# Kkuntal990/video-to-video-diffusion

Hardware: AMD Instinct MI355X
Metric: ddim_steps_per_sec (higher is better)
Workload: dtype bf16; 1 GPU; DDIM-50 step (U-Net eval + update) on latent [1, 8, 48, 128, 128] = 8->48 slices @512x512, effective 264.66M U-Net (128x(1,2,4,4), latent 8), one volume per GPU, hipGraph-captured step; volumes_per_gpu=1, parallelism=dp1, full=False, finite_outputs=True

## Files before the change

video-to-video-diffusion_amd/csrc/conv_mfma.hip:

```cpp
#include <type_traits>
#include "conv3_halo_common.h"
#include "conv_plan.h"
#include <string.h>
#include <stdlib.h>
#include <math.h>


__device__ __attribute__((aligned(256))) uint32_t g_ctsi_zero_page[64];

struct ConvKParams {
    const bf16_t* x1;
    const bf16_t* x2;
    const bf16_t* w;
    const float* bias;
    void* y;
    float* colsum;
    int C1, C2, Cin;
    int Di, Hi, Wi;
    int Dr, Hr, Wr;
    int sH, sW;
    int lTH, lTW;
    int linear;
    int tilesD, tilesH, tilesW, tps, mtiles;
    int ntiles_n;
// ... 470 lines not shown
            const int co = n0 + col;
            float s1 = 0.0f, s2 = 0.0f;
#pragma unroll
            for (int i = 0; i < TM; ++i) {
#pragma unroll
                for (int r = 0; r < 16; ++r) {
                    const int row = wm * TM * 32 + i * 32 + (r & 3) + 8 * (r >> 2) + 4 * lhi;
                    float v = acc[i][j][r];
                    if (p.act == 1) v = tanhf(v);
                    const bool valid = (vbits[i] >> r) & 1u;
                    if (valid) {
                        s1 += v;
                        s2 += v * v;
                    }
                    if (p.out_mode == 0) {
                        s_tile[row * BN + col] = f32_to_bf16(v);
                    } else if (valid && co < p.Cout) {
                        reinterpret_cast<float*>(p.y)[s_rowoff[row] + (long long)co * p.osc] = v;
                    }
                }
            }
            if (want_sums) {
                s1 += __shfl_xor(s1, 32);
                s2 += __shfl_xor(s2, 32);
                if (lhi == 0) {
                    s_cs[(wm * BN + col) * 2 + 0] = s1;
                    s_cs[(wm * BN + col) * 2 + 1] = s2;
                }
            }
        }
    }
    if (p.gn_x != nullptr && tid < BN) {
        const int co = n0 + tid;
        float sc = 0.0f, sh = 0.0f;
        if (co < p.Cout) {
            const int cpg = p.Cout / p.gn_groups, g = co / cpg;
            const double* sm = p.gn_sums + ((long long)nb * p.gn_groups + g) * 2;
            const double mean = sm[0] / p.gn_count;
            double var = sm[1] / p.gn_count - mean * mean;
            if (var < 0.0) var = 0.0;
            const float rstd = (float)(1.0 / sqrt(var + (double)p.gn_eps));
            sc = p.gn_gamma[co] * rstd;
            sh = p.gn_beta[co] - (float)mean * sc;
        }
        s_cs[tid] = sc;
        s_cs[BN + tid] = sh;
    }
    __syncthreads();
    if (p.colsum != nullptr && tid < BN) {
        float t1 = 0.0f, t2 = 0.0f;
#pragma unroll
        for (int m = 0; m < WM; ++m) {
            t1 += s_cs[(m * BN + tid) * 2 + 0];
            t2 += s_cs[(m * BN + tid) * 2 + 1];
        }
        const long long tg = (long long)cls * p.mtiles + mt;
        const long long slab = (long long)p.nclass * p.mtiles * p.CoutPad;
        p.colsum[tg * p.CoutPad + n0 + tid] = t1;
        p.colsum[slab + tg * p.CoutPad + n0 + tid] = t2;
    }
    if (p.out_mode == 0) {
        constexpr int CPR = BN / 8;
        constexpr int ITER = (BM * CPR) / NTH;
        static_assert((BM * CPR) % NTH == 0, "store loop assumes whole iterations");
        bf16_t* y = reinterpret_cast<bf16_t*>(p.y);
        if (p.gn_x != nullptr) {
            uint4 hreg[ITER];
#pragma unroll
            for (int it = 0; it < ITER; ++it) {
                const int c = tid + it * NTH;
                const int row = c / CPR, cc = c - row * CPR;
                const long long off = s_rowoff[row];
                const int co = n0 + cc * 8;
                hreg[it] = (off >= 0 && co < p.Cout) ? *reinterpret_cast<const uint4*>(p.gn_x + off + co)
                                                     : make_uint4(0, 0, 0, 0);
            }
            static_assert(NTH % CPR == 0, "a thread's chunk must not depend on the iteration");
            const int cc0 = tid % CPR;
            float gsc[8], gsh[8];
            *reinterpret_cast<float4*>(gsc) = *reinterpret_cast<const float4*>(s_cs + cc0 * 8);
            *reinterpret_cast<float4*>(gsc + 4) = *reinterpret_cast<const float4*>(s_cs + cc0 * 8 + 4);
            *reinterpret_cast<float4*>(gsh) = *reinterpret_cast<const float4*>(s_cs + BN + cc0 * 8);
            *reinterpret_cast<float4*>(gsh + 4) = *reinterpret_cast<const float4*>(s_cs + BN + cc0 * 8 + 4);
            auto tail = [&](auto silu_tag) {
                constexpr bool SILU = decltype(silu_tag)::value;
#pragma unroll
                for (int it = 0; it < ITER; ++it) {
                    const int c = tid + it * NTH;
                    const int row = c / CPR, cc = c - row * CPR;
                    const long long off = s_rowoff[row];
                    const int co = n0 + cc * 8;
                    if (off >= 0 && co < p.Cout) {
                        const uint4 v = *reinterpret_cast<const uint4*>(s_tile + row * BN + cc * 8);
                        const uint4 h = hreg[it];
                        const uint32_t hw[4] = {h.x, h.y, h.z, h.w}, rw[4] = {v.x, v.y, v.z, v.w};
                        uint32_t ow[4];
#pragma unroll
                        for (int k = 0; k < 4; ++k) {
                            f32x2_t a = {__uint_as_float(hw[k] << 16), __uint_as_float(hw[k] & 0xffff0000u)};
                            a = a * f32x2_t{gsc[2 * k], gsc[2 * k + 1]} + f32x2_t{gsh[2 * k], gsh[2 * k + 1]} +
                                f32x2_t{__uint_as_float(rw[k] << 16), __uint_as_float(rw[k] & 0xffff0000u)};
                            if (SILU) a = silu2_f(a);
                            ow[k] = pack_bf16x2_v(a);
                        }
                        *reinterpret_cast<uint4*>(y + off + co) = make_uint4(ow[0], ow[1], ow[2], ow[3]);
                    }
                }
            };
            if (p.gn_silu) tail(std::true_type{});
            else tail(std::false_type{});
        } else {
            for (int c = tid; c < BM * CPR; c += NTH) {
                const int row = c / CPR, cc = c - row * CPR;
                const long long off = s_rowoff[row];
                const int co = n0 + cc * 8;
                if (off >= 0 && co < p.Cout && !(CTSI_DBG_RT(p.dbg, 1))) {
                    const uint4 v = *reinterpret_cast<const uint4*>(s_tile + row * BN + cc * 8);
                    *reinterpret_cast<uint4*>(y + off + co) = v;
                }
            }
        }
    }
#endif
}

struct PackParams {
    const float* w;
    bf16_t* out;
    int nclass, T, Cout, CoutPad, Cin, CinW, Ktot, small, kc_per_tap, lcpt;
    long long s_co, s_ci;
    int tapk[CTSI_MAX_TAPS];
};

__global__ void conv_pack_weights_kernel(const PackParams q) {
    const long long total = (long long)q.nclass * q.CoutPad * q.Ktot;
    for (long long idx = (long long)blockIdx.x * blockDim.x + threadIdx.x; idx < total;
         idx += (long long)gridDim.x * blockDim.x) {
        const int k = (int)(idx % q.Ktot);
        const long long rc = idx / q.Ktot;
        const int co = (int)(rc % q.CoutPad);
        const int cls = (int)(rc / q.CoutPad);
        int tap, ci;
        if (q.small) {
            const int g = k >> 3;
            tap = g >> q.lcpt;
            ci = ((g & ((1 << q.lcpt) - 1)) << 3) + (k & 7);
        } else {
            const int s = k >> 6;
            tap = s % q.T;
            ci = (s / q.T) * 64 + (k & 63);
        }
        float v = 0.0f;
        if (tap < q.T && ci < q.CinW && co < q.Cout)
            v = q.w[(long long)co * q.s_co + (long long)ci * q.s_ci + q.tapk[cls * q.T + tap]];
        q.out[idx] = f32_to_bf16(v);
    }
}

extern "C" int ctsi_conv_plan_pack_weights(const ctsi_conv_plan* p, const float* w, void* packed,
                                           void* stream) {
    CTSI_CHECK_ARG(p && w && packed, "ctsi_conv_plan_pack_weights: null argument");
    if (p->stem) return ctsi_conv3_stem_pack(w, packed, p->d.cout, p->CoutPad, p->CinW, stream);
    if (p->stream1) return ctsi_conv1_stream_pack(w, packed, p->d.cout, p->Cin, p->CinW, p->stream1, stream);
    const ConvFamily family = conv_family(p);
    if (family == CONV_K32)
        return ctsi_conv3_halo_k32_pack(w, packed, p->d.cout, p->CoutPad, p->Cin, p->CinW, p->BN, conv_k32_image(p),
                                        conv_k32_direct(p), stream);
    if (family == CONV_HEAD) {
        hipMemsetAsync((char*)packed + head1_bytes(p) - 1280, 0, 1280, (hipStream_t)stream);
        if (ctsi_conv3_head2_supported(p->Cin, p->d.cout)) {
            const int rc = ctsi_conv3_head2_pack(w, (char*)packed + head1_bytes(p), p->d.cout, p->Cin, p->CinW, stream);
            if (rc != CTSI_OK) return rc;
        }
        return ctsi_conv3_halo_pack(w, packed, p->d.cout, p->d.cout <= 8 ? 8 : 16, p->Cin, p->CinW, stream);
    }
    if (family == CONV_HALO32) return ctsi_conv3_halo_pack(w, packed, p->d.cout, p->CoutPad, p->Cin, p->CinW, stream);
    PackParams q;
    memset(&q, 0, sizeof(q));
    q.w = w;
    q.out = (bf16_t*)packed;
    q.nclass = p->nclass;
    q.T = p->T;
    q.Cout = p->d.cout;
    q.CoutPad = p->CoutPad;
    q.Cin = p->Cin;
    q.CinW = p->CinW;
    q.Ktot = p->Ktot;
    q.small = p->small;
    q.kc_per_tap = p->kc_per_tap;
    q.lcpt = p->lcpt;
    const long long KK = (long long)p->d.kd * p->d.kh * p->d.kw;
    if (!p->d.transposed) {
        q.s_co = (long long)p->CinW * KK;
        q.s_ci = KK;
    } else {
        q.s_ci = (long long)p->d.cout * KK;
        q.s_co = KK;
    }
    memcpy(q.tapk, p->tapk, sizeof(q.tapk));
    const long long total = (long long)q.nclass * q.CoutPad * q.Ktot;
    const int blocks = (int)((total + 255) / 256 > 4096 ? 4096 : (total + 255) / 256);
    hipLaunchKernelGGL(conv_pack_weights_kernel, dim3(blocks), dim3(256), 0, (hipStream_t)stream, q);
    CTSI_LAUNCH_CHECK();
    return CTSI_OK;
}

template <int WM, int WN, int TM, int TN>
static int launch_conv(const ConvKParams& k, int mode, int grid, hipStream_t st) {
    constexpr int BM = WM * TM * 32, BN = WN * TN * 32;
    constexpr size_t lds = 2 * (BM * 128 + BN * 128) + BM * 8 + WM * BN * 8;
    constexpr int STAGE = BM * 128 + BN * 128;
    constexpr int NSTG = STAGE <= 32768 ? 4 : (STAGE <= 49152 ? 3 : 2);
    constexpr size_t lds_ring = (size_t)NSTG * STAGE + BM * 8 + WM * BN * 8;
    static CtsiPerDeviceOnce attr_once;
    if (attr_once.first()) {
        hipFuncSetAttribute((const void*)conv_gather_mfma_kernel<WM, WN, TM, TN, 3>,
                            hipFuncAttributeMaxDynamicSharedMemorySize, (int)lds_ring);
        hipFuncSetAttribute((const void*)conv_gather_mfma_kernel<WM, WN, TM, TN, 0>,
                            hipFuncAttributeMaxDynamicSharedMemorySize, (int)lds);
        hipFuncSetAttribute((const void*)conv_gather_mfma_kernel<WM, WN, TM, TN, 1>,
                            hipFuncAttributeMaxDynamicSharedMemorySize, (int)lds);
        hipFuncSetAttribute((const void*)conv_gather_mfma_kernel<WM, WN, TM, TN, 2>,
                            hipFuncAttributeMaxDynamicSharedMemorySize, (int)lds);
    }
    const dim3 g(grid), b(WM * WN * 64);
    if (mode == 1)
        hipLaunchKernelGGL((conv_gather_mfma_kernel<WM, WN, TM, TN, 1>), g, b, lds, st, k);
    else if (mode == 3)
        hipLaunchKernelGGL((conv_gather_mfma_kernel<WM, WN, TM, TN, 3>), g, b, lds_ring, st, k);
    else if (mode == 2)
        hipLaunchKernelGGL((conv_gather_mfma_kernel<WM, WN, TM, TN, 2>), g, b, lds, st, k);
    else
        hipLaunchKernelGGL((conv_gather_mfma_kernel<WM, WN, TM, TN, 0>), g, b, lds, st, k);
    CTSI_LAUNCH_CHECK();
    return CTSI_OK;
}

extern "C" int ctsi_conv_fwd(const ctsi_conv_plan* p, const void* x1, const void* x2, const void* packed_w,
                             const float* bias, const ctsi_conv_out* o, void* stream) {
    CTSI_CHECK_ARG(p && x1 && packed_w && o && o->y, "ctsi_conv_fwd: null argument");
    CTSI_CHECK_ARG(p->d.c2 == 0 || x2 != nullptr, "ctsi_conv_fwd: plan has two sources but x2 is null");
    CTSI_CHECK_ARG(o->mode == 0 || o->mode == 1, "ctsi_conv_fwd: bad output mode %d", o->mode);
    if (o->mode == 0) {
        CTSI_CHECK_ARG(p->d.cout % 8 == 0 && o->cout_stride % 8 == 0 && o->c_off % 8 == 0 &&
                           o->cout_stride >= o->c_off + p->d.cout,
                       "ctsi_conv_fwd: bf16 output needs cout, cout_stride, c_off multiples of 8 "
                       "(cout=%d stride=%d off=%d)", p->d.cout, o->cout_stride, o->c_off);
    }
    const ConvFamily family = conv_family(p);
    CTSI_CHECK_ARG(o->act != 2 || (p->planar && o->mode == 0 && o->colsum == nullptr && o->gn_x == nullptr),
                   "ctsi_conv_fwd: the ReLU epilogue (act = 2) exists on planar (1,3,3) halo-tile plans with plain bf16 output "
                   "only (ctsi_conv_plan_form: bit 16 of out[4])");
    CTSI_CHECK_ARG(!p->planar || o->colsum == nullptr, "ctsi_conv_fwd: a planar (1,3,3) halo-tile plan writes no column sums");
    if (p->stem && o->mode == 0 && o->act == 0 && o->gn_x == nullptr) {
        StemParams q;
        memset(&q, 0, sizeof(q));
        q.x = (const bf16_t*)x1;
        q.w = (const bf16_t*)packed_w;
        q.bias = bias;
        q.y = (bf16_t*)o->y;
        q.colsum = (float*)o->colsum;
        q.cx = p->d.c1;
        q.D = p->d.di; q.H = p->d.hi; q.W = p->d.wi;
        q.Cout = p->d.cout; q.CoutPad = p->CoutPad;
        q.cout_stride = o->cout_stride; q.c_off = o->c_off;
        q.tilesD = p->tilesD; q.tilesH = p->tilesH; q.tilesW = p->tilesW; q.tps = p->tps; q.mtiles = p->mtiles;
        return ctsi_conv3_stem_launch(&q, stream);
    }
    CTSI_CHECK_ARG(!p->stem, "ctsi_conv_fwd: a one-channel stem plan writes bf16 without activation or fused tail");
    if (p->stream1) {
        CTSI_CHECK_ARG(o->mode == 0 && o->act == 0 && o->colsum == nullptr,
                       "ctsi_conv_fwd: a streaming 1x1x1 plan writes bf16 without activation or column sums");
        Conv1StreamParams q;
        memset(&q, 0, sizeof(q));
        q.x1 = (const bf16_t*)x1;
        q.x2 = (const bf16_t*)(x2 ? x2 : x1);
        q.w = (const bf16_t*)packed_w;
        q.bias = bias;
        q.h = (const bf16_t*)o->gn_x;
        q.y = (bf16_t*)o->y;
        if (o->gn_x != nullptr) {
            CTSI_CHECK_ARG(o->gn_sums && o->gn_gamma && o->gn_beta && o->gn_groups > 0 && p->d.cout % o->gn_groups == 0 &&
                               o->gn_count > 0,
                           "ctsi_conv_fwd: bad fused GroupNorm arguments (groups=%d, cout=%d)", o->gn_groups, p->d.cout);
            q.gn_sums = (const double*)o->gn_sums;
            q.gn_gamma = (const float*)o->gn_gamma;
            q.gn_beta = (const float*)o->gn_beta;
            q.gn_groups = o->gn_groups;
            q.gn_eps = o->gn_eps;
            q.gn_count = (double)o->gn_count;
            q.gn_silu = o->gn_silu;
        }
        q.C1 = p->d.c1; q.C2 = p->d.c2; q.Cout = p->d.cout;
        q.cout_stride = o->cout_stride; q.c_off = o->c_off;
        q.V = (long long)p->Do * p->Ho * p->Wo;
        return ctsi_conv1_stream_launch(&q, p->d.n, p->stream1, stream);
    }
    if (o->gn_x != nullptr) {
        CTSI_CHECK_ARG(!p->form && o->mode == 0 && o->act == 0 && o->colsum == nullptr && p->nclass == 1,
                       "ctsi_conv_fwd: the fused GroupNorm tail needs a gather-kernel plan, bf16 output, no act / colsum");
        CTSI_CHECK_ARG(o->gn_sums && o->gn_gamma && o->gn_beta && o->gn_groups > 0 && p->d.cout % o->gn_groups == 0 &&
                           o->gn_count > 0,
                       "ctsi_conv_fwd: bad fused GroupNorm arguments (groups=%d, cout=%d)", o->gn_groups, p->d.cout);
    }
    if (p->form && (family == CONV_HEAD || (o->mode == 0 && (o->act == 0 || o->act == 2)))) {
        Conv3HaloParams h;
        memset(&h, 0, sizeof(h));
        h.x1 = (const bf16_t*)x1;
        h.x2 = (const bf16_t*)(x2 ? x2 : x1);
        h.w = (const bf16_t*)packed_w;
        h.bias = bias;
        h.y = o->y;
        h.colsum = o->colsum;
        h.C1 = p->d.c1; h.C2 = p->d.c2;
        h.Di = p->d.di; h.Hi = p->d.hi; h.Wi = p->d.wi;
        h.Do = p->Do; h.Ho = p->Ho; h.Wo = p->Wo;
        h.dshift = p->dshift;
        h.tilesD = p->tilesD; h.tilesH = p->tilesH; h.tilesW = p->tilesW; h.tps = p->tps; h.mtiles = p->mtiles;
        h.ntiles_n = p->ntiles_n;
        h.nchunks = p->Cin / (family == CONV_K32 ? 16 : 32) * (p->ds ? 4 : 1);
        h.ds = p->ds;
        h.Cout = p->d.cout; h.CoutPad = p->CoutPad;
        h.cout_stride = o->cout_stride; h.c_off = o->c_off;
        {
            static const char* nts = getenv("CTSI_CONV_NT_STORE");
            const long long out_bytes = (long long)p->d.n * p->Do * p->Ho * p->Wo * o->cout_stride * 2;
            h.nt_store = nts ? atoi(nts) != 0 : out_bytes >= (128ll << 20);
        }
        {
            const char* nm = getenv("CTSI_CONV_NMAJOR");
            h.n_major = nm ? atoi(nm) : 0;
            if (p->d.transposed && !nm) h.n_major = 4;
        }
        {
            h.dbg = ctsi_debug_flags();
            h.nchunks = ctsi_debug_ksteps(h.nchunks);
        }
        {
            const char* to = getenv("CTSI_CONV_TILE_ORDER");
            h.tile_order = to ? atoi(to) : 2;
            const char* eb = getenv("CTSI_CONV_EPI_BARRIER");
            h.dbg_epi_barrier = eb ? atoi(eb) : 0;
        }
        if (family == CONV_HEAD) {
            if (p->head2 && o->colsum == nullptr)
                return ctsi_conv3_head2_launch(&h, p->d.n, (const char*)packed_w + head1_bytes(p), o->mode, o->act, o->sn, o->sc, o->sd,
                                               o->sh, o->sw, stream);
            return ctsi_conv3_head_launch(&h, p->d.cout <= 8 ? 8 : 16, o->mode, o->act, o->sn, o->sc, o->sd, o->sh, o->sw, stream);
        }
        h.tr = p->d.transposed;
        if (family == CONV_K32 && p->ksplit == 2) {
            CTSI_CHECK_ARG(o->workspace, "ctsi_conv_fwd: this plan needs ctsi_conv_out.workspace (ctsi_conv_plan_workspace_bytes)");
            const int tiles = p->mtiles * p->ntiles_n;
            h.ksplit = 2;
            h.sk_sync = (int*)o->workspace;
            h.sk_ws = (float*)((char*)o->workspace + ((size_t)tiles * 8 + 255) / 256 * 256);
        }
        if (p->planar) return ctsi_conv3_planar_k32_launch(&h, p->form->code, o->act == 2, stream);
        if (family == CONV_K32) return ctsi_conv3_halo_k32_launch(&h, p->form->code, p->BN, stream);
        return ctsi_conv3_halo_launch(&h, p->form->code, stream);
    }
    CTSI_CHECK_ARG(!p->form, "ctsi_conv_fwd: the 3x3x3 halo-tile plan supports bf16 NDHWC output without activation");
    ConvKParams k;
    memset(&k, 0, sizeof(k));
    k.x1 = (const bf16_t*)x1;
    k.x2 = (const bf16_t*)(x2 ? x2 : x1);
    k.w = (const bf16_t*)packed_w;
    k.bias = bias;
    k.y = o->y;
    k.colsum = o->colsum;
    k.C1 = p->d.c1; k.C2 = p->d.c2; k.Cin = p->Cin;
    k.Di = p->d.di; k.Hi = p->d.hi; k.Wi = p->d.wi;
    k.Dr = p->Dr; k.Hr = p->Hr; k.Wr = p->Wr;
    k.sH = p->sH; k.sW = p->sW;
    k.lTH = p->lTH; k.lTW = p->lTW;
    k.linear = p->linear;
    k.tilesD = p->tilesD; k.tilesH = p->tilesH; k.tilesW = p->tilesW; k.tps = p->tps; k.mtiles = p->mtiles;
    k.ntiles_n = p->ntiles_n;
    k.T = p->T; k.ksteps = p->ksteps; k.kc_per_tap = p->kc_per_tap; k.lcpt = p->lcpt;
    k.Cout = p->d.cout; k.CoutPad = p->CoutPad; k.Ktot = p->Ktot;
    k.Do = p->Do; k.Ho = p->Ho; k.Wo = p->Wo; k.uH = p->uH; k.uW = p->uW;
    k.nclass = p->nclass;
    k.out_mode = o->mode; k.cout_stride = o->cout_stride; k.c_off = o->c_off; k.act = o->act;
    k.osn = o->sn; k.osc = o->sc; k.osd = o->sd; k.osh = o->sh; k.osw = o->sw;
    memcpy(k.tapdelta, p->tapdelta, sizeof(k.tapdelta));
    k.NA = p->NA; k.NB = p->NB; k.NC = p->NC;
    memcpy(k.ad, p->ad, sizeof(k.ad));
    memcpy(k.bh, p->bh, sizeof(k.bh));
    memcpy(k.cw, p->cw, sizeof(k.cw));
    for (int c = 0; c < 4; ++c) { k.pH[c] = p->pH[c]; k.pW[c] = p->pW[c]; }
    int grid = p->nclass * p->mtiles * p->ntiles_n;
    if (p->gsplit >= 2 && o->workspace != nullptr && !(p->BM != 128 || p->BN != 128)) {
        const size_t tiles = (size_t)grid;
        k.ksplit = p->gsplit;
        k.sk_sync = (int*)o->workspace;
        k.sk_ws = (float*)((char*)o->workspace + (tiles * 4 + 255) / 256 * 256);
        grid *= p->gsplit;
    }
    hipStream_t st = (hipStream_t)stream;
    k.ksteps = ctsi_debug_ksteps(k.ksteps);
    k.dbg = ctsi_debug_flags();
    k.gn_x = (const bf16_t*)o->gn_x;
    k.gn_sums = o->gn_sums;
    k.gn_gamma = o->gn_gamma;
    k.gn_beta = o->gn_beta;
    k.gn_groups = o->gn_groups;
    k.gn_silu = o->gn_silu;
    k.gn_eps = o->gn_eps;
    k.gn_count = (double)o->gn_count;
    k.dshift = p->dshift;
    memcpy(k.tap_margin, p->tap_margin, sizeof(k.tap_margin));
    memcpy(k.ad_min, p->ad_min, sizeof(k.ad_min));
    int mode = p->small ? 1 : (p->fast ? 2 : 0);
    {
        const char* ring = getenv("CTSI_CONV_RING");
        const bool small_grid = grid <= 256 && !(p->BM == 256 && p->BN == 256);
        if (mode == 2 && ((small_grid && !(ring && !strcmp(ring, "0"))) || (ring && !strcmp(ring, "1")))) mode = 3;
    }
    if (p->BM == 256 && p->BN == 256) return launch_conv<2, 4, 4, 2>(k, mode, grid, st);
    if (p->BM == 256 && p->BN == 128) return launch_conv<4, 2, 2, 2>(k, mode, grid, st);
    if (p->BN == 128) return launch_conv<2, 2, 2, 2>(k, mode, grid, st);
    return launch_conv<4, 1, 1, 1>(k, mode, grid, st);
}
```

video-to-video-diffusion_amd/csrc/ctsi_internal.h:

```cpp
#pragma once
#include <hip/hip_runtime.h>
#include <stdint.h>
#include <stdio.h>
#include <stdarg.h>
#include "../../include/ctsi.h"

typedef uint16_t bf16_t;

typedef __attribute__((ext_vector_type(8))) short bf16x8;
typedef __attribute__((ext_vector_type(4))) float f32x4;
typedef __attribute__((ext_vector_type(16))) float f32x16;

void ctsi_set_error(const char* fmt, ...);

#define CTSI_CHECK_ARG(cond, ...)            \
    do {                                     \
        if (!(cond)) {                       \
            ctsi_set_error(__VA_ARGS__);     \
            return CTSI_ERR_INVALID;         \
        }                                    \
    } while (0)

struct CtsiPerDeviceOnce {
    bool done[64] = {};
    bool first() {
        int d = 0;
        if (hipGetDevice(&d) != hipSuccess || d < 0 || d >= 64) return true;
        if (done[d]) return false;
        done[d] = true;
        return true;
    }
};

#define CTSI_HIP(call)                                                                  \
    do {                                                                                \
        hipError_t e_ = (call);                                                         \
        if (e_ != hipSuccess) {                                                         \
            ctsi_set_error("%s failed: %s (%s:%d)", #call, hipGetErrorString(e_),       \
                           __FILE__, __LINE__);                                         \
            return CTSI_ERR_HIP;                                                        \
        }                                                                               \
    } while (0)

#define CTSI_LAUNCH_CHECK()                                                             \
    do {                                                                                \
        hipError_t e_ = hipGetLastError();                                              \
        if (e_ != hipSuccess) {                                                         \
            ctsi_set_error("kernel launch failed: %s (%s:%d)", hipGetErrorString(e_),   \
                           __FILE__, __LINE__);                                         \
            return CTSI_ERR_HIP;                                                        \
        }                                                                               \
    } while (0)

#ifdef CTSI_ABLATE
#define CTSI_DBG(flags, bit) ((flags) & (bit))
#define CTSI_DBG_MASK (~0)
#else
#define CTSI_DBG(flags, bit) (((bit) == 4096) ? ((flags) & 4096) : 0)
#define CTSI_DBG_MASK 4096
#endif
#define CTSI_DBG_RT(flags, bit) ((flags) & (bit))
int ctsi_debug_flags();
int ctsi_debug_ksteps(int n);

__device__ __forceinline__ float bf16_to_f32(bf16_t v) {
    return __uint_as_float(((uint32_t)v) << 16);
}
__device__ __forceinline__ bf16_t f32_to_bf16(float f) {
    __bf16 b = (__bf16)f;
    return *reinterpret_cast<bf16_t*>(&b);
}
__device__ __forceinline__ uint32_t pack_bf16x2(float lo, float hi) {
    return (uint32_t)f32_to_bf16(lo) | ((uint32_t)f32_to_bf16(hi) << 16);
}
__device__ __forceinline__ float silu_f(float x) {
    return x * __builtin_amdgcn_rcpf(1.0f + __builtin_amdgcn_exp2f(-1.4426950408889634f * x));
}

typedef float f32x2_t __attribute__((ext_vector_type(2)));
typedef __bf16 bf16x2_t __attribute__((ext_vector_type(2)));
__device__ __forceinline__ f32x2_t silu2_f(f32x2_t x) {
    f32x2_t t = x * -1.4426950408889634f;
    t.x = __builtin_amdgcn_exp2f(t.x);
    t.y = __builtin_amdgcn_exp2f(t.y);
    t = 1.0f + t;
    t.x = __builtin_amdgcn_rcpf(t.x);
    t.y = __builtin_amdgcn_rcpf(t.y);
    return x * t;
}
__device__ __forceinline__ uint32_t pack_bf16x2_v(f32x2_t v) {
    const bf16x2_t b = __builtin_convertvector(v, bf16x2_t);
    return *reinterpret_cast<const uint32_t*>(&b);
}

__device__ __forceinline__ float nan_to_num_f(float v) {
    if (v != v) return 0.0f;
    if (v == __builtin_inff()) return 1.0f;
    if (v == -__builtin_inff()) return -1.0f;
    return v;
}

static inline int ceil_div(int a, int b) { return (a + b - 1) / b; }

struct Conv3HaloParams {
    const bf16_t* x1;
    const bf16_t* x2;
    const bf16_t* w;
    const float* bias;
    void* y;
    float* colsum;
    int C1, C2;
    int Di, Hi, Wi;
    int Do, Ho, Wo;
    int dshift;
    int tilesD, tilesH, tilesW, tps, mtiles, ntiles_n;
    int nchunks;
    int Cout, CoutPad;
    int cout_stride, c_off;
    int n_major;
    int dbg;
    const double* nin_sums;
    const float* nin_gamma;
    const float* nin_beta;
    const float* nin_tbias;
    const int* nin_step_ptr;
    int nin_tb_stride, nin_groups, nin_silu, nin_n_total;
    int nin_pad_lo, nin_pad_hi;
    float nin_eps;
    double nin_count;
    int ksplit;
    float* sk_ws;
    int* sk_sync;
    int tr;
    int ds;
    int tile_order;
    int nt_store;
    int dbg_epi_barrier;
};

extern "C" int ctsi_conv3_halo_pack(const float* w, void* packed, int cout, int cout_pad, int cin, int cin_w,
                                    void* stream);
extern "C" int ctsi_conv3_halo_launch(const Conv3HaloParams* hp, int wide, void* stream);
extern "C" int ctsi_conv3_head_launch(const Conv3HaloParams* hp, int rows, int out_mode, int act, long long sn, long long sc,
                                      long long sd, long long sh, long long sw, void* stream);
extern "C" int ctsi_conv3_head2_supported(int cin, int cout);
extern "C" size_t ctsi_conv3_head2_weight_bytes(int cout);
extern "C" int ctsi_conv3_head2_pack(const float* w, void* packed, int cout, int cin, int cin_w, void* stream);
extern "C" int ctsi_conv3_head2_launch(const Conv3HaloParams* hp, int n, const void* packed, int out_mode, int act, long long sn,
                                       long long sc, long long sd, long long sh, long long sw, void* stream);
struct StemParams {
    const bf16_t* x;
    const bf16_t* w;
    const float* bias;
    bf16_t* y;
    float* colsum;
    int cx, D, H, W;
    int Cout, CoutPad, cout_stride, c_off;
    int tilesD, tilesH, tilesW, tps, mtiles;
};
extern "C" void ctsi_conv3_stem_tile(int* td, int* th, int* tw);
extern "C" size_t ctsi_conv3_stem_weight_bytes(int cout_pad);
extern "C" int ctsi_conv3_stem_pack(const float* w, void* packed, int cout, int cout_pad, int cin_w, void* stream);
extern "C" int ctsi_conv3_stem_launch(const StemParams* q, void* stream);

struct Conv1StreamParams {
    const bf16_t* x1;
    const bf16_t* x2;
    const bf16_t* w;
    const float* bias;
    const bf16_t* h;
    bf16_t* y;
    const double* gn_sums;
    const float* gn_gamma;
    const float* gn_beta;
    int gn_groups, gn_silu;
    float gn_eps;
    double gn_count;
    int C1, C2, Cout, cout_stride, c_off;
    long long V;
    int tiles;
    int P;
};
extern "C" int ctsi_conv1_stream_switch();
extern "C" int ctsi_conv1_stream_nt(int c1, int c2, int cout);
extern "C" int ctsi_conv1_stream_pack(const float* w, void* packed, int cout, int cin, int cin_w, int nt, void* stream);
extern "C" int ctsi_conv1_stream_launch(Conv1StreamParams* q, int n, int nt, void* stream);
extern "C" size_t ctsi_conv3_halo_k32_weight_bytes(int cin, int cout_pad, int bn, int transposed);
extern "C" int ctsi_conv3_halo_k32_pack(const float* w, void* packed, int cout, int cout_pad, int cin, int cin_w, int bn,
                                        int transposed, int direct, void* stream);
extern "C" int ctsi_conv3_halo_k32_direct(int tile, int ksplit, int ds);
extern "C" size_t ctsi_conv3_halo_k32_splitk_bytes(int tiles);
extern "C" int ctsi_conv3_halo_k32_launch(const Conv3HaloParams* hp, int tile, int bn, void* stream);
extern "C" int ctsi_conv3_planar_k32_launch(const Conv3HaloParams* hp, int tile, int relu, void* stream);
```

Baseline: 40.25 steps/s.

## Add persistent pipelined 1x1 conv kernel with fused GroupNorm residual epilogue

Measured after the change: 40.36 steps/s (median of 6 runs). About the same (+0.3%).

```diff
diff --git a/video-to-video-diffusion_amd/csrc/conv1_pipe.hip b/video-to-video-diffusion_amd/csrc/conv1_pipe.hip
--- /dev/null
+++ b/video-to-video-diffusion_amd/csrc/conv1_pipe.hip
@@ -0,0 +1,288 @@
+#include "conv3_halo_common.h"
+#include <stdlib.h>
+#include <type_traits>
+
+namespace {
+
+constexpr int C1P_TM = 2;
+constexpr int C1P_BM = 2 * C1P_TM * 32;
+constexpr int C1P_BN = 256;
+constexpr int C1P_NSTG = 3;
+constexpr int C1P_STAGE = (C1P_BM + C1P_BN) * 128;
+constexpr int C1P_LDS = C1P_NSTG * C1P_STAGE + 3 * C1P_BN * 4;
+
+__device__ __forceinline__ v4i_t c1p_load16(const bf16_t* ptr) {
+    v4i_t v;
+    asm volatile("global_load_dwordx4 %0, %1, off" : "=v"(v) : "v"(ptr) : "memory");
+    return v;
+}
+
+#define C1P_WAIT(N) asm volatile("s_waitcnt vmcnt(%0)" ::"n"(N) : "memory")
+
+}
+
+__global__ void __launch_bounds__(512)
+conv1_pipe_kernel(const Conv1PipeParams p) {
+#if defined(__HIP_DEVICE_COMPILE__)
+    constexpr int TM = C1P_TM, TN = 2, BM = C1P_BM, BN = C1P_BN, NSTG = C1P_NSTG, STAGE = C1P_STAGE;
+    constexpr int A_BYTES = BM * 128;
+    constexpr int A_INSTR = BM / 64, B_INSTR = BN / 64, DPS = A_INSTR + B_INSTR;
+    constexpr int HL = TM * TN * 2;
+    static_assert(HL == 8, "the wait on the h registers lists them one by one");
+
+    extern __shared__ __attribute__((aligned(16))) char smem[];
+    float* s_bias = reinterpret_cast<float*>(smem + NSTG * STAGE);
+    float* s_sc = s_bias + BN;
+    float* s_sh = s_sc + BN;
+
+    const int tid = threadIdx.x;
+    const int lane = tid & 63;
+    const int wave = __builtin_amdgcn_readfirstlane(tid >> 6);
+    const int wm = wave >> 2, wn = wave & 3;
+    const int lhi = lane >> 5, lcol = lane & 31;
+    const int nt = blockIdx.y, nb = blockIdx.z;
+    const int n0 = nt * BN;
+    const int P = gridDim.x;
+    const int tiles = p.tiles;
+    const int S = p.Ktot >> 6;
+    const int C1 = p.C1, C2 = p.C2;
+    const long long V = p.V;
+
+    if (tid < BN) {
+        const int co = n0 + tid;
+        const int cpg = p.Cout / p.gn_groups, g = co / cpg;
+        const double* sm = p.gn_sums + ((long long)nb * p.gn_groups + g) * 2;
+        const double mean = sm[0] / p.gn_count;
+        double var = sm[1] / p.gn_count - mean * mean;
+        if (var < 0.0) var = 0.0;
+        const float rstd = (float)(1.0 / sqrt(var + (double)p.gn_eps));
+        const float sc = p.gn_gamma[co] * rstd;
+        s_bias[tid] = p.bias != nullptr ? p.bias[co] : 0.0f;
+        s_sc[tid] = sc;
+        s_sh[tid] = p.gn_beta[co] - (float)mean * sc;
+    }
+    __syncthreads();
+
+    const v4i_t rr1 = h3_make_rsrc(p.x1 + (long long)nb * V * C1, 0x7fffffffu);
+    const v4i_t rr2 = h3_make_rsrc(p.x2 + (long long)nb * V * C2, 0x7fffffffu);
+    const v4i_t rrw = h3_make_rsrc(p.w + (long long)n0 * p.Ktot, 0x7fffffffu);
+    const unsigned lds0 = (unsigned)(unsigned long long)(lptr3_t)smem;
+    int a_row[A_INSTR];
+    unsigned a_q16[A_INSTR];
+#pragma unroll
+    for (int i = 0; i < A_INSTR; ++i) {
+        a_row[i] = (wave * A_INSTR + i) * 8 + (lane >> 3);
+        a_q16[i] = (unsigned)(((lane & 7) ^ ((a_row[i] >> 1) & 7)) * 16);
+    }
+    unsigned b_voff[B_INSTR];
+#pragma unroll
+    for (int i = 0; i < B_INSTR; ++i) {
+        const int m = (wave * B_INSTR + i) * 8 + (lane >> 3);
+        const int m5 = m & 31, mh = (m5 >> 2) & 1, mr = (m5 & 3) + 4 * (m5 >> 3);
+        const int co = (m & ~31) + mh * 8 + (mr & 7) + 16 * (mr >> 3);
+        b_voff[i] = (unsigned)co * (unsigned)(p.Ktot * 2) + (unsigned)(((lane & 7) ^ ((m >> 1) & 7)) * 16);
+    }
+    int st_tile = blockIdx.x, st_k = 0;
+    unsigned a_v1[A_INSTR], a_v2[A_INSTR];
+    auto set_rows = [&](int tile) {
+#pragma unroll
+        for (int i = 0; i < A_INSTR; ++i) {
+            const long long row = (long long)tile * BM + a_row[i];
+            const bool ok = tile < tiles && row < V;
+            a_v1[i] = ok ? (unsigned)row * (unsigned)(C1 * 2) + a_q16[i] : 0x80000000u;
+            a_v2[i] = ok ? (unsigned)row * (unsigned)(C2 * 2) + a_q16[i] : 0x80000000u;
+        }
+    };
+    auto stage = [&](int slot) {
+        const int ch0 = st_k * 64;
+        const bool second = ch0 >= C1;
+        const unsigned soff = (unsigned)__builtin_amdgcn_readfirstlane((second ? ch0 - C1 : ch0) * 2);
+        const unsigned abase = lds0 + slot * STAGE + wave * (A_INSTR * 1024);
+#pragma unroll
+        for (int i = 0; i < A_INSTR; ++i) {
+            const unsigned dst = (unsigned)__builtin_amdgcn_readfirstlane((int)(abase + i * 1024));
+            if (second)
+                h3_dma16(rr2, dst, a_v2[i], soff);
+            else
+                h3_dma16(rr1, dst, a_v1[i], soff);
+        }
+        const unsigned bbase = lds0 + slot * STAGE + A_BYTES + wave * (B_INSTR * 1024);
+        const unsigned wsoff = (unsigned)__builtin_amdgcn_readfirstlane(st_k * 128);
+#pragma unroll
+        for (int i = 0; i < B_INSTR; ++i) {
+            const unsigned dst = (unsigned)__builtin_amdgcn_readfirstlane((int)(bbase + i * 1024));
+            h3_dma16(rrw, dst, b_voff[i], wsoff);
+        }
+        if (++st_k == S) {
+            st_k = 0;
+            st_tile += P;
+            set_rows(st_tile);
+        }
+    };
+
+    const int fsw = (lane >> 1) & 7;
+    int koff[4];
+#pragma unroll
+    for (int kk = 0; kk < 4; ++kk) koff[kk] = (((kk * 2 + lhi) ^ fsw) << 4) + lcol * 128;
+    f32x16 acc[TM][TN];
+    auto compute = [&](const char* cur) {
+        const char* x_base = cur + (wm * TM * 32) * 128;
+        const char* w_base = cur + A_BYTES + (wn * TN * 32) * 128;
+#pragma unroll
+        for (int kk = 0; kk < 4; ++kk) {
+            bf16x8 xf[TM], wf[TN];
+#pragma unroll
+            for (int i = 0; i < TM; ++i) xf[i] = *reinterpret_cast<const bf16x8*>(x_base + i * 32 * 128 + koff[kk]);
+#pragma unroll
+            for (int j = 0; j < TN; ++j) wf[j] = *reinterpret_cast<const bf16x8*>(w_base + j * 32 * 128 + koff[kk]);
+#pragma unroll
+            for (int i = 0; i < TM; ++i)
+#pragma unroll
+                for (int j = 0; j < TN; ++j)
+                    acc[i][j] = __builtin_amdgcn_mfma_f32_32x32x16_bf16(wf[j], xf[i], acc[i][j], 0, 0, 0);
+        }
+    };
+
+    const int cbase = wn * (TN * 32) + lhi * 8;
+    const long long ch_off = (long long)p.c_off + n0 + cbase;
+    v4i_t hr[HL];
+    auto issue_h = [&](int tile) {
+#pragma unroll
+        for (int i = 0; i < TM; ++i) {
+            long long row = (long long)tile * BM + wm * (TM * 32) + i * 32 + lcol;
+            row = row < V ? row : V - 1;
+            const bf16_t* ph = p.h + ((long long)nb * V + row) * p.cout_stride + ch_off;
+#pragma unroll
+            for (int j = 0; j < TN; ++j)
+#pragma unroll
+                for (int q = 0; q < 2; ++q) hr[(i * TN + j) * 2 + q] = c1p_load16(ph + j * 32 + q * 16);
+        }
+    };
+    auto epilogue = [&](int tile, auto full_tag, auto silu_tag) {
+        constexpr bool FULL = decltype(full_tag)::value, SILU = decltype(silu_tag)::value;
+#pragma unroll
+        for (int j = 0; j < TN; ++j)
+#pragma unroll
+            for (int q = 0; q < 2; ++q) {
+                float gsc[8], gsh[8];
+                const int c = cbase + j * 32 + q * 16;
+                *reinterpret_cast<float4*>(gsc) = *reinterpret_cast<const float4*>(s_sc + c);
+                *reinterpret_cast<float4*>(gsc + 4) = *reinterpret_cast<const float4*>(s_sc + c + 4);
+                *reinterpret_cast<float4*>(gsh) = *reinterpret_cast<const float4*>(s_sh + c);
+                *reinterpret_cast<float4*>(gsh + 4) = *reinterpret_cast<const float4*>(s_sh + c + 4);
+#pragma unroll
+                for (int i = 0; i < TM; ++i) {
+                    const long long row = (long long)tile * BM + wm * (TM * 32) + i * 32 + lcol;
+                    const v4i_t h = hr[(i * TN + j) * 2 + q];
+                    const uint32_t hw[4] = {(uint32_t)h.x, (uint32_t)h.y, (uint32_t)h.z, (uint32_t)h.w};
+                    uint32_t ow[4];
+#pragma unroll
+                    for (int k = 0; k < 4; ++k) {
+                        const uint32_t rw = pack_bf16x2_v(f32x2_t{acc[i][j][q * 8 + 2 * k], acc[i][j][q * 8 + 2 * k + 1]});
+                        f32x2_t a = {__uint_as_float(hw[k] << 16), __uint_as_float(hw[k] & 0xffff0000u)};
+                        a = a * f32x2_t{gsc[2 * k], gsc[2 * k + 1]} + f32x2_t{gsh[2 * k], gsh[2 * k + 1]} +
+                            f32x2_t{__uint_as_float(rw << 16), __uint_as_float(rw & 0xffff0000u)};
+                        if (SILU) a = silu2_f(a);
+                        ow[k] = pack_bf16x2_v(a);
+                    }
+                    bf16_t* py = p.y + ((long long)nb * V + (FULL || row < V ? row : 0)) * p.cout_stride + ch_off + j * 32 + q * 16;
+                    if (FULL || row < V) *reinterpret_cast<uint4*>(py) = make_uint4(ow[0], ow[1], ow[2], ow[3]);
+                }
+            }
+    };
+
+    set_rows(st_tile);
+    stage(0);
+    stage(1);
+    int slot = 0;
+    bool first = true;
+    for (int tile = blockIdx.x; tile < tiles; tile += P) {
+#pragma unroll
+        for (int j = 0; j < TN; ++j) {
+            float bv[16];
+#pragma unroll
+            for (int q = 0; q < 4; ++q)
+                *reinterpret_cast<float4*>(bv + 4 * q) = *reinterpret_cast<const float4*>(s_bias + cbase + j * 32 + (q >> 1) * 16 + (q & 1) * 4);
+#pragma unroll
+            for (int i = 0; i < TM; ++i)
+#pragma unroll
+                for (int r = 0; r < 16; ++r) acc[i][j][r] = bv[r];
+        }
+        auto step = [&](auto h_tag) {
+            __builtin_amdgcn_s_barrier();
+            stage(slot == 0 ? NSTG - 1 : slot - 1);
+            if (decltype(h_tag)::value) issue_h(tile);
+            compute(smem + slot * STAGE);
+            asm volatile("s_waitcnt lgkmcnt(0)" ::: "memory");
+            slot = (slot + 1 == NSTG) ? 0 : slot + 1;
+        };
+#pragma nounroll
+        for (int k = 0; k < S - 3; ++k) {
+            if (k < 2 && !first) C1P_WAIT(DPS + HL);
+            else C1P_WAIT(DPS);
+            step(std::false_type{});
+        }
+        C1P_WAIT(DPS);
+        step(std::true_type{});
+        C1P_WAIT(DPS + HL);
+        step(std::false_type{});
+        C1P_WAIT(DPS + HL);
+        step(std::false_type{});
+        asm volatile("s_waitcnt vmcnt(%8)"
+                     : "+v"(hr[0]), "+v"(hr[1]), "+v"(hr[2]), "+v"(hr[3]), "+v"(hr[4]), "+v"(hr[5]), "+v"(hr[6]), "+v"(hr[7])
+                     : "n"(2 * DPS)
+                     : "memory");
+        const bool full = (long long)(tile + 1) * BM <= V;
+        using T = std::true_type;
+        using F = std::false_type;
+        if (full) {
+            if (p.gn_silu) epilogue(tile, T{}, T{});
+            else epilogue(tile, T{}, F{});
+        } else {
+            if (p.gn_silu) epilogue(tile, F{}, T{});
+            else epilogue(tile, F{}, F{});
+        }
+        first = false;
+    }
+    asm volatile("s_waitcnt vmcnt(0)" ::: "memory");
+#endif
+}
+
+extern "C" int ctsi_conv1_pipe_enabled() {
+    const char* e = getenv("CTSI_CONV1_PIPE");
+    return e ? atoi(e) != 0 : 1;
+}
+
+extern "C" int ctsi_conv1_pipe_supported(int c1, int c2, int cout, long long voxels) {
+    const int k = c1 + c2, cmax = c1 > c2 ? c1 : c2;
+    return c1 > 0 && c1 % 64 == 0 && c2 % 64 == 0 && k >= 768 && cout % C1P_BN == 0 && voxels > 0 &&
+           (double)voxels * cmax * 2.0 < 2.0e9 && (voxels + C1P_BM - 1) / C1P_BM < (1ll << 30);
+}
+
+static long long g_c1p_launches = 0;
+extern "C" long long ctsi_conv1_pipe_launches() { return g_c1p_launches; }
+
+extern "C" int ctsi_conv1_pipe_launch(Conv1PipeParams* q, int n, void* stream) {
+    CTSI_CHECK_ARG(q && q->h && ctsi_conv1_pipe_supported(q->C1, q->C2, q->Cout, q->V) && q->Ktot == q->C1 + q->C2,
+                   "ctsi_conv1_pipe_launch: unsupported layer");
+    q->tiles = (int)((q->V + C1P_BM - 1) / C1P_BM);
+    static int cus = 0;
+    if (!cus) {
+        int dev = 0, v = 0;
+        if (hipGetDevice(&dev) == hipSuccess && hipDeviceGetAttribute(&v, hipDeviceAttributeMultiprocessorCount, dev) == hipSuccess && v > 0)
+            cus = v;
+        else
+            cus = 256;
+    }
+    const int ntn = q->Cout / C1P_BN;
+    const char* fb = getenv("CTSI_CONV1_PIPE_BLOCKS");
+    int P = (fb && atoi(fb) > 0 ? atoi(fb) : cus) / (ntn * n);
+    if (P > q->tiles) P = q->tiles;
+    if (P < 1) P = 1;
+    static CtsiPerDeviceOnce attr_once;
+    if (attr_once.first()) hipFuncSetAttribute((const void*)conv1_pipe_kernel, hipFuncAttributeMaxDynamicSharedMemorySize, C1P_LDS);
+    hipLaunchKernelGGL(conv1_pipe_kernel, dim3(P, ntn, n), dim3(512), C1P_LDS, (hipStream_t)stream, *q);
+    CTSI_LAUNCH_CHECK();
+    ++g_c1p_launches;
+    return CTSI_OK;
+}
diff --git a/video-to-video-diffusion_amd/csrc/conv_mfma.hip b/video-to-video-diffusion_amd/csrc/conv_mfma.hip
--- a/video-to-video-diffusion_amd/csrc/conv_mfma.hip
+++ b/video-to-video-diffusion_amd/csrc/conv_mfma.hip
@@ -796,8 +796,35 @@
         CTSI_CHECK_ARG(o->gn_sums && o->gn_gamma && o->gn_beta && o->gn_groups > 0 && p->d.cout % o->gn_groups == 0 &&
                            o->gn_count > 0,
                        "ctsi_conv_fwd: bad fused GroupNorm arguments (groups=%d, cout=%d)", o->gn_groups, p->d.cout);
-    }
-    if (p->form && (family == CONV_HEAD || (o->mode == 0 && (o->act == 0 || o->act == 2)))) {
+        const bool splitk = p->gsplit >= 2 && o->workspace != nullptr && p->BM == 128 && p->BN == 128;
+        const long long vox = (long long)p->Do * p->Ho * p->Wo;
+        if (p->fast && !p->small && p->T == 1 && !p->d.transposed && p->dshift == 0 && p->sH == 1 && p->sW == 1 &&
+            p->uH == 1 && p->uW == 1 && p->Ktot == p->d.c1 + p->d.c2 && p->d.di == p->Do && p->d.hi == p->Ho && p->d.wi == p->Wo && p->Dr == p->Do &&
+            p->Hr == p->Ho && p->Wr == p->Wo && p->pH[0] == 0 && p->pW[0] == 0 && !splitk &&
+            ctsi_debug_flags() == 0 && ctsi_debug_ksteps(p->ksteps) == p->ksteps && ctsi_conv1_pipe_enabled() &&
+            ctsi_conv1_pipe_supported(p->d.c1, p->d.c2, p->d.cout, vox)) {
+            Conv1PipeParams q;
+            memset(&q, 0, sizeof(q));
+            q.x1 = (const bf16_t*)x1;
+            q.x2 = (const bf16_t*)(x2 ? x2 : x1);
+            q.w = (const bf16_t*)packed_w;
+            q.bias = bias;
+            q.h = (const bf16_t*)o->gn_x;
+            q.y = (bf16_t*)o->y;
+            q.gn_sums = (const double*)o->gn_sums;
+            q.gn_gamma = (const float*)o->gn_gamma;
+            q.gn_beta = (const float*)o->gn_beta;
+            q.gn_groups = o->gn_groups;
+            q.gn_silu = o->gn_silu;
+            q.gn_eps = o->gn_eps;
+            q.gn_count = (double)o->gn_count;
+            q.C1 = p->d.c1; q.C2 = p->d.c2; q.Cout = p->d.cout; q.Ktot = p->Ktot;
+            q.cout_stride = o->cout_stride; q.c_off = o->c_off;
+            q.V = vox;
+            return ctsi_conv1_pipe_launch(&q, p->d.n, stream);
+        }
+    }
+    if (p->form &&(family == CONV_HEAD || (o->mode == 0 && (o->act == 0 || o->act == 2)))) {
         Conv3HaloParams h;
         memset(&h, 0, sizeof(h));
         h.x1 = (const bf16_t*)x1;
diff --git a/video-to-video-diffusion_amd/csrc/ctsi_internal.h b/video-to-video-diffusion_amd/csrc/ctsi_internal.h
--- a/video-to-video-diffusion_amd/csrc/ctsi_internal.h
+++ b/video-to-video-diffusion_amd/csrc/ctsi_internal.h
@@ -185,6 +185,27 @@
 extern "C" int ctsi_conv1_stream_nt(int c1, int c2, int cout);
 extern "C" int ctsi_conv1_stream_pack(const float* w, void* packed, int cout, int cin, int cin_w, int nt, void* stream);
 extern "C" int ctsi_conv1_stream_launch(Conv1StreamParams* q, int n, int nt, void* stream);
+struct Conv1PipeParams {
+    const bf16_t* x1;
+    const bf16_t* x2;
+    const bf16_t* w;
+    const float* bias;
+    const bf16_t* h;
+    bf16_t* y;
+    const double* gn_sums;
+    const float* gn_gamma;
+    const float* gn_beta;
+    int gn_groups, gn_silu;
+    float gn_eps;
+    double gn_count;
+    int C1, C2, Cout, Ktot, cout_stride, c_off;
+    long long V;
+    int tiles;
+};
+extern "C" int ctsi_conv1_pipe_enabled();
+extern "C" int ctsi_conv1_pipe_supported(int c1, int c2, int cout, long long voxels);
+extern "C" int ctsi_conv1_pipe_launch(Conv1PipeParams* q, int n, void* stream);
+extern "C" long long ctsi_conv1_pipe_launches();
 extern "C" size_t ctsi_conv3_halo_k32_weight_bytes(int cin, int cout_pad, int bn, int transposed);
 extern "C" int ctsi_conv3_halo_k32_pack(const float* w, void* packed, int cout, int cout_pad, int cin, int cin_w, int bn,
                                         int transposed, int direct, void* stream);
```
